# tomwhite/disq

Hardware: AMD Instinct MI355X
Metric: decompressed BAM GB/s + reads/sec (whole node) at 1/2/4/8 MI355X (higher is better)
Workload: dtype u8

## Files before the change

disq_amd/csrc/dq_hdr_core.h:

```cpp
#pragma once
#include <stdint.h>

#ifndef __HIPCC__
#ifndef __host__
#define __host__
#define __device__
#endif
#endif

#define DQH_INLINE __host__ __device__ inline __attribute__((always_inline))

namespace dqh {

enum : int32_t {
  HDR_NONE = 0,
  HDR_DYN = 1,
  HDR_ERR = 2,
};
constexpr int32_t HDR_BAD_TABLE = 4, HDR_OVERREAD = 8;
constexpr uint32_t HDR_WORDS = 160;
constexpr int HDR_LENS = 320;

struct HdrInfo {
  int32_t kind, status;
  int32_t nlen, ndist, bfinal;
  uint32_t end;
};

template <class Src>
struct Bits {
  uint64_t bb;
  uint32_t bc, wp;
  DQH_INLINE void init(const Src& S, uint32_t pos) {
    const uint32_t wi = pos >> 5, sh = pos & 31;
    bb = (((uint64_t)S.word(wi + 1) << 32) | S.word(wi)) >> sh;
    bc = 64 - sh;
    wp = wi + 2;
  }
  DQH_INLINE void fill(const Src& S) {
    if (bc <= 32) {
      bb |= (uint64_t)S.word(wp) << bc;
      bc += 32;
      wp += 1;
    }
  }
  DQH_INLINE uint32_t peek() const { return (uint32_t)bb; }
  DQH_INLINE void skip(uint32_t n) {
    bb >>= n;
    bc -= n;
  }
  DQH_INLINE uint32_t pos() const { return wp * 32 - bc; }
};

template <class Src, class Tbl, class Sink>
DQH_INLINE HdrInfo hdr_decode(const Src& S, Tbl& T, Sink& K, uint32_t pos, uint32_t endbits) {
  constexpr uint8_t order[19] = {16, 17, 18, 0, 8, 7, 9, 6, 10, 5, 11, 4, 12, 3, 13, 2, 14, 1, 15};
  HdrInfo R = {HDR_NONE, 0, 0, 0, 0, pos};
  if (pos + 3 > endbits) return R;
  Bits<Src> B;
  B.init(S, pos);
  const uint32_t h = B.peek();
  R.bfinal = (int32_t)(h & 1);
  if (((h >> 1) & 3) != 2) return R;
  R.nlen = (int32_t)((h >> 3) & 31) + 257;
  R.ndist = (int32_t)((h >> 8) & 31) + 1;
  const int ncode = (int)((h >> 13) & 15) + 4;
  B.skip(17);
  R.kind = HDR_ERR;
  R.status = HDR_BAD_TABLE;
  if (R.nlen > 286 || R.ndist > 30) return R;
  if (pos + 17 + 3 * (uint32_t)ncode > endbits) {
    R.status = HDR_OVERREAD;
    return R;
  }
  uint64_t cl = 0, cnt = 0;
  for (int i = 0; i < 19; i++) {
    B.fill(S);
    const uint32_t v = i < ncode ? B.peek() & 7 : 0;
    B.skip(i < ncode ? 3 : 0);
    cl |= (uint64_t)v << (3 * order[i]);
    cnt += 1ull << (8 * v);
  }
  uint64_t nxt = 0;
  {
    int left = 1;
    uint32_t code = 0;
    bool ok = true;
    for (int l = 1; l <= 7; l++) {
      const int c = (int)((cnt >> (8 * l)) & 0xff);
      left = 2 * left - c;
      ok = ok && left >= 0;
      nxt |= (uint64_t)(code & 0xff) << (8 * l);
      code = (code + (uint32_t)c) << 1;
    }
    if (!ok || left != 0) return R;
  }
  for (int s = 0; s < 19; s++) {
    const uint32_t l = (uint32_t)(cl >> (3 * s)) & 7;
    if (l == 0) continue;
    const uint32_t c = (uint32_t)(nxt >> (8 * l)) & 0xff;
    nxt += 1ull << (8 * l);
    uint32_t r = 0;
    for (uint32_t i = 0; i < l; i++) r |= ((c >> i) & 1u) << (l - 1 - i);
    for (uint32_t k = r & 127; k < 128; k += 1u << l) T.set(k, (uint32_t)s << 3 | l);
  }
  const int total = R.nlen + R.ndist;
  int have = 0, prev = -1;
  bool eob = false;
  for (int it = 0; it < 316 && have < total; it++) {
    if (B.pos() > endbits) {
      R.status = HDR_OVERREAD;
      return R;
    }
    B.fill(S);
    const uint32_t v = B.peek();
    const uint32_t e = T.get(v & 127);
    const uint32_t len = e & 7, sy = e >> 3;
    if (len == 0) return R;
    const uint32_t ex = sy < 16 ? 0u : sy == 16 ? 2u : sy == 17 ? 3u : 7u;
    const int xv = (int)((v >> len) & ((1u << ex) - 1));
    B.skip(len + ex);
    const int rep = sy < 16 ? 1 : sy == 18 ? 11 + xv : 3 + xv;
    const int val = sy < 16 ? (int)sy : sy == 16 ? prev : 0;
    if (val < 0) return R;
    if (have + rep > total) return R;
    if (val != 0)
      for (int i = have; i < have + rep; i++) {
        K.put((uint32_t)(i < R.nlen ? i : 288 + i - R.nlen), (uint32_t)val);
        eob = eob || i == 256;
      }
    have += rep;
    prev = val;
  }
  if (have < total) return R;
  R.end = B.pos();
  if (R.end > endbits) {
    R.status = HDR_OVERREAD;
    return R;
  }
  if (!eob) return R;
  R.kind = HDR_DYN;
  R.status = 0;
  return R;
}

}
```

disq_amd/csrc/dq_inflate3.hip:

```cpp
#include "dq_hdr_core.h"
#include "dq_inflate_core.h"
#include "dq_internal.h"

#include <mutex>
#include <vector>

namespace dq {
namespace {

using namespace dqi;

#define DQ_HD __device__ __host__ __attribute__((always_inline)) inline

#ifndef DQ_BLK_WG
#define DQ_BLK_WG 512
#endif
constexpr int WG = DQ_BLK_WG;
static_assert(WG % 128 == 0 && WG >= 512 && WG <= 1024, "whole waves on every SIMD");
constexpr int NWV = WG / 64;
constexpr int NDEC = WG;
constexpr uint32_t OV_DEFAULT = 96;
#ifndef DQ_TAIL_OV
#define DQ_TAIL_OV OV_DEFAULT
#endif
// ... 1370 lines not shown
    }
    int32_t msv[NE];
    uint32_t da[NB], db[NB];
#pragma unroll
    for (int k = 0; k < NB; k++) {
      const int32_t g0 = b0 + k * CH + G * t;
#pragma unroll
      for (int i = 0; i < G; i++) {
        const uint64_t mi = mw[k] & (~0ull >> (63 - ((g0 + i) & 63)));
        msv[k * G + i] = mi ? (g0 | 63) - (int32_t)__clzll(mi) : lsv[k];
      }
      da[k] = load_desc(L, sh + min(msv[k * G], 65535));
      db[k] = G > 1 ? load_desc(L, sh + min(msv[k * G + G - 1], 65535)) : da[k];
    }
#pragma unroll
    for (int k = 0; k < NB; k++) {
      const int32_t g0 = b0 + k * CH + G * t;
      const int32_t sbk = b0 + k * CH + (CSTEP ? 0 : ((G * t) & ~511));
#pragma unroll
      for (int i = 0; i < G; i++) {
        const int e = k * G + i;
        const int32_t x = g0 + i, ms = msv[e];
        const bool before = ms < b0;
        const uint32_t desc = before ? cdesc : (ms == msv[k * G + G - 1] ? db[k] : da[k]);
        const int32_t len = (int32_t)(desc >> 15) + 3, D1 = (int32_t)(desc & 0x7fff);
        const bool copy = x < rsize && ms != 0xffff && (!before || ms == cms) && x < ms + len;
        const int32_t jj = x - ms;
        int32_t src = (int32_t)((uint32_t)D1 ^ ~0u) + x;
        if (__builtin_expect(__any(copy && jj > D1), 0)) {
          const int32_t D = D1 + 1;
          const int32_t q = (int32_t)((float)jj * __builtin_amdgcn_rcpf((float)D));
          int32_t r = jj - q * D;
          r = r >= D ? r - D : r;
          src = ms - D + r;
        }
        DQ_CHK(!copy || (src >= 0 && src < x), CHK_K2_SRC);
        const bool done = !copy || src < sbk;
        fr[e] = copy ? src : x;
        xs[e] = done ? x : src;
        pending = pending || !done;
        nxt[x - b0] = (uint16_t)(copy ? src : x);
      }
    }
  };
  auto jump_round = [&](int32_t b0, int32_t* fr, int32_t* xs, bool& pending) {
    int32_t qv[NE];
#pragma unroll
    for (int e = 0; e < NE; e++) {
      DQ_CHK(xs[e] - b0 >= 0 && xs[e] - b0 < BATCH, CHK_K2_NXT);
      qv[e] = (int32_t)zx16(nxt[xs[e] - b0]);
    }
    bool any = false;
#pragma unroll
    for (int e = 0; e < NE; e++) {
      const int32_t own = (e / G) * CH + G * t + e % G;
      const int32_t p = xs[e], q = qv[e];
      const bool pd = p != b0 + own;
      const int32_t sbk = b0 + (e / G) * CH + (CSTEP ? 0 : ((G * t) & ~511));
      const bool fin = pd && (q == p || q < sbk);
      const bool go = pd && !fin;
      fr[e] = fin ? q : fr[e];
      xs[e] = go ? q : b0 + own;
      any = any || go;
      if constexpr (!QUAD) nxt[own] = (uint16_t)q;
    }
    if constexpr (QUAD) {
#pragma unroll
      for (int k = 0; k < NB; k++)
        store_nxt4(k * CH + 4 * t, pack16(qv[4 * k], qv[4 * k + 1]), pack16(qv[4 * k + 2], qv[4 * k + 3]));
    }
    pending = any;
  };
  constexpr bool SLICE = DQ_RES_SLICE != 0;
  const uint32_t own2 = 2u * (uint32_t)t;
  auto LB = [](int e) { return 2u << e; };
  auto nxt_at = [&](int e, uint32_t ra) {
    return reinterpret_cast<uint16_t*>(reinterpret_cast<char*>(nxt) + e * (CH * 2) + ra);
  };
  auto adopt_live = [&](int32_t b0, int32_t* fr, uint32_t* ra, uint32_t& live) {
    int32_t qv[NE];
#pragma unroll
    for (int e = 0; e < NE; e++) qv[e] = (int32_t)zx16(*nxt_at(e, own2));
    const uint32_t cb = 2u * (uint32_t)-b0;
    live = 0;
    uint64_t anym = 0;
#pragma unroll
    for (int e = 0; e < NE; e++) {
      const uint32_t na = ((uint32_t)qv[e] << 1) + (cb - 2u * e * CH);
      const bool pend = na < own2;
      fr[e] = qv[e];
      ra[e] = pend ? na : own2;
      if constexpr (SLICE) live |= __ballot(pend) != 0 ? LB(e) : 0u;
      else anym |= __ballot(pend);
    }
    if constexpr (!SLICE) live = anym != 0 ? LB(0) : 0u;
  };
  auto jump_round_live = [&](int32_t b0, int32_t* fr, uint32_t* ra, uint32_t& live) {
    const uint32_t cb = 2u * (uint32_t)-b0;
#pragma unroll
    for (int e = 0; e < NE; e++)
      if (!SLICE || (live & LB(e))) {
        DQ_CHK(ra[e] < 2u * CH && !(ra[e] & 1u), CHK_K2_NXT);
        fr[e] = *nxt_at(e, ra[e]);
      }
    uint32_t nl = 0;
    uint64_t anym = 0;
#pragma unroll
    for (int e = 0; e < NE; e++)
      if (!SLICE || (live & LB(e))) {
        const uint32_t q = zx32(fr[e]);
        fr[e] = (int32_t)q;
        const uint32_t na = (q << 1) + (cb - 2u * e * CH);
        const bool pd = ra[e] != own2, lt = na < ra[e];
        ra[e] = pd && lt ? na : own2;
        if constexpr (SLICE) nl |= (__ballot(pd) & __ballot(lt)) != 0 ? LB(e) : 0u;
        else anym |= __ballot(pd) & __ballot(lt);
        *nxt_at(e, own2) = (uint16_t)q;
      }
    live = SLICE ? nl : anym != 0 ? LB(0) : 0u;
  };
  int32_t frA[NE], xsA[NE];
  uint32_t raA[NE];
  bool pendA = false;
  uint32_t liveA = 0;
  auto left = [&](bool pending, uint32_t live) { return HYB ? live != 0 : pending; };
  auto round = [&](int32_t b0, int32_t* fr, int32_t* xs, uint32_t* ra, bool& pending, uint32_t& live) {
    if constexpr (HYB) jump_round_live(b0, fr, ra, live);
    else jump_round(b0, fr, xs, pending);
  };
  int32_t cms = -1;
  uint32_t cdesc = 0;
  first_hop(0, cms, cdesc, frA, xsA, pendA);
  if (t < (rsize + BATCH - 1) / BATCH) {
    int32_t ncms = -1;
    uint32_t ncdesc = 0;
    const int32_t x = (t + 1) * BATCH - 1;
    if (x + 1 < rsize) {
      const uint64_t m = bm64[x >> 6];
      const int32_t ms = m ? (x | 63) - (int32_t)__clzll(m) : (int32_t)L.u.r.last_start[(x >> 6) - 1];
      if (ms != 0xffff) {
        const uint32_t desc = load_desc(L, sh + ms);
        if (ms + (int32_t)(desc >> 15) + 3 > x + 1) {
          ncms = ms;
          ncdesc = desc;
        }
      }
    }
    L.u.r.carry_ms[t] = ncms;
    L.u.r.carry_desc[t] = ncdesc;
  }
  __syncthreads();
  if constexpr (HYB) adopt_live(0, frA, raA, liveA);
  for (int hop = 0; left(pendA, liveA) && hop < WG + 2; hop++) round(0, frA, xsA, raA, pendA, liveA);
  const int32_t rsize_u = HYB ? __builtin_amdgcn_readfirstlane(rsize) : rsize;
  for (int32_t bs = 0; bs < rsize_u; bs += BATCH) {
    const uint64_t tb0 = TIMING ? __builtin_amdgcn_s_memtime() : 0;
    const int32_t nbs = bs + BATCH;
    const bool more = nbs < rsize_u;
    __syncthreads();
    const int32_t ncms = more ? L.u.r.carry_ms[bs / BATCH] : -1;
    const uint32_t ncdesc = more ? L.u.r.carry_desc[bs / BATCH] : 0u;
    int32_t frB[NE], xsB[NE];
    uint32_t raB[NE];
    bool pendB = false;
    uint32_t liveB = 0;
    if (more) first_hop(nbs, ncms, ncdesc, frB, xsB, pendB);
    const uint64_t tb1 = TIMING ? __builtin_amdgcn_s_memtime() : 0;
#pragma unroll
    for (int k = 0; k < NB; k++) {
#pragma unroll
      for (int j = 0; j < (CSTEP ? 1 : G); j++) {
        const bool mine = CSTEP || ((G * t) >> 9) == j;
        const int32_t g0 = bs + k * CH + G * t;
        uint8_t v[G];
        if (mine)
#pragma unroll
          for (int i = 0; i < G; i++) {
            DQ_CHK(g0 + i >= rsize || (frA[k * G + i] >= 0 && frA[k * G + i] <= g0 + i), CHK_K2_SRC);
            v[i] = O[INR ? frA[k * G + i] : min(frA[k * G + i], 65535)];
          }
        if constexpr (HYB)
          if (k == 1 && more) adopt_live(nbs, frB, raB, liveB);
        if ((k > 0 || j > 0) && left(pendB, liveB)) round(nbs, frB, xsB, raB, pendB, liveB);
        if constexpr (QUAD && INR) {
          if (mine) {
            const uint32_t lo = (uint32_t)v[0] | (uint32_t)v[1] << 8;
            const uint32_t hi = (uint32_t)v[2] | (uint32_t)v[3] << 8;
            uint8_t* const p = L.out + sh + g0;
            if ((sh & 3) == 0) {
              const uint32_t w4 = lo | hi << 16;
              __builtin_memcpy(__builtin_assume_aligned(p, 4), &w4, 4);
            } else if ((sh & 3) == 2) {
              const uint16_t a2 = (uint16_t)lo, b2 = (uint16_t)hi;
              __builtin_memcpy(__builtin_assume_aligned(p, 2), &a2, 2);
              __builtin_memcpy(__builtin_assume_aligned(p + 2, 2), &b2, 2);
            } else {
              const uint16_t m2 = (uint16_t)(v[1] | v[2] << 8);
              p[0] = v[0];
              __builtin_memcpy(__builtin_assume_aligned(p + 1, 2), &m2, 2);
              p[3] = v[3];
            }
          }
        } else {
          if (mine)
#pragma unroll
            for (int i = 0; i < G; i++)
              if (g0 + i < rsize) L.out[sh + g0 + i] = v[i];
        }
        __syncthreads();
      }
    }
    if (left(pendB, liveB)) round(nbs, frB, xsB, raB, pendB, liveB);
    const uint64_t tb2 = TIMING ? __builtin_amdgcn_s_memtime() : 0;
    const int32_t c1 = min(rsize, nbs);
    const int32_t lines_to = c1 >= head ? (c1 - head) / 16 : 0;
    if (!(sflags & 1)) {
      for (int32_t k = lines_done + t; k < lines_to; k += WG) {
        const uint4 v = *reinterpret_cast<const uint4*>(O + head + 16 * k);
        uint4* d = reinterpret_cast<uint4*>(dstU + head + 16 * k);
        if (sflags & 2) st_nt(d, v);
        else *d = v;
      }
      lines_done = lines_to;
    }
    const uint64_t tb3 = TIMING ? __builtin_amdgcn_s_memtime() : 0;
    for (int hop = 0; left(pendB, liveB) && hop < WG + 2; hop++) round(nbs, frB, xsB, raB, pendB, liveB);
#pragma unroll
    for (int e = 0; e < NE; e++) frA[e] = frB[e];
    cms = ncms;
    cdesc = ncdesc;
    if (TIMING && t == 0) {
      tacc[9] += tb1 - tb0;
      tacc[12] += tb2 - tb1;
      tacc[13] += tb3 - tb2;
      tacc[14] += __builtin_amdgcn_s_memtime() - tb3;
      tacc[15] += 1;
    }
  }
  if (sflags & 1) {
    const int32_t lines_to = rsize >= head ? (rsize - head) / 16 : 0;
    for (int32_t k = t; k < lines_to; k += WG) {
      const uint4 v = *reinterpret_cast<const uint4*>(O + head + 16 * k);
      uint4* d = reinterpret_cast<uint4*>(dstU + head + 16 * k);
      if (sflags & 2) st_nt(d, v);
      else *d = v;
    }
    lines_done = lines_to;
  }
  uint32_t ct0 = 0, ct1 = 0, cshift = 0, cinit = 0, cwant = 0;
  if (verify_crc) {
    ct0 = (&c_crc4[0][0])[t];
    ct1 = t + WG < 1024 ? (&c_crc4[0][0])[t + WG] : 0u;
    cshift = c_slice_shift[WG - 1 - t];
    if (t == 0) {
      cinit = crc_init[rsize];
      const uint8_t* tr = C + cpos + csize - 8;
      cwant = (uint32_t)tr[0] | ((uint32_t)tr[1] << 8) | ((uint32_t)tr[2] << 16) | ((uint32_t)tr[3] << 24);
    }
  }
  static_assert(2 * WG >= 1024, "at most two CRC table words per thread");
  for (int x = t; x < head; x += WG) dstU[x] = O[x];
  for (int x = head + 16 * lines_done + t; x < rsize; x += WG) dstU[x] = O[x];
  TST(6);
  if (verify_crc) {
    __syncthreads();
    if (t < 1024) (&L.u.crc4[0][0])[t] = ct0;
    if (t + WG < 1024) (&L.u.crc4[0][0])[t + WG] = ct1;
    __syncthreads();
    const int32_t e = rsize - (WG - 1 - t) * CRC_SL;
    const int32_t s0 = max(0, e - CRC_SL);
    uint32_t cr = 0;
    if (e > 0) {
      int32_t x = s0;
      while (x < e && ((sh + x) & 3)) cr = L.u.crc4[0][(cr ^ O[x++]) & 0xff] ^ (cr >> 8);
      for (; x + 4 <= e; x += 4) {
        const uint32_t v = cr ^ *reinterpret_cast<const uint32_t*>(O + x);
        cr = L.u.crc4[3][v & 0xff] ^ L.u.crc4[2][(v >> 8) & 0xff] ^ L.u.crc4[1][(v >> 16) & 0xff] ^
             L.u.crc4[0][v >> 24];
      }
      while (x < e) cr = L.u.crc4[0][(cr ^ O[x++]) & 0xff] ^ (cr >> 8);
      cr = gf2_mulmod(cshift, cr);
    }
    cr = wave_incl_xor(cr);
    if (lane == 63) L.wsum[wv] = (int32_t)cr;
    __syncthreads();
    if (t == 0) {
      uint32_t x = 0;
      for (int w = 0; w < WG / 64; w++) x ^= (uint32_t)L.wsum[w];
      if (deferred) {
        tails[blockIdx.x].crc_raw = x;
      } else {
        const uint32_t crc = (x ^ cinit) ^ 0xffffffffu;
        if (crc != cwant) status[b] = ST_CRC;
      }
    }
  }
  TST(7);
  if (TIMING && t == 0)
    for (int i = 0; i < 24; i++) tim[(int64_t)blockIdx.x * TIM_W + i] = tacc[i];
  if (TIMING && t == 0)
    for (int i = 0; i < 7; i++) tim[(int64_t)blockIdx.x * TIM_W + 24 + i] = (uint64_t)L.misc[21 + i];
}

constexpr int HP_LS = 65;
struct HpSrc {
  const uint32_t* __restrict__ W;
  uint32_t last;
  DQ_AI uint32_t word(uint32_t i) const {
    return *reinterpret_cast<const uint32_t*>(reinterpret_cast<const uint8_t*>(W) + (min(i, last) << 2));
  }
};
struct HpTbl {
  uint8_t* t;
  DQ_AI void set(uint32_t k, uint32_t v) { t[k * 64] = (uint8_t)v; }
  DQ_AI uint32_t get(uint32_t k) const { return t[k * 64]; }
};
struct HpSink {
  uint32_t* w;
  uint32_t cur, acc;
  DQ_AI void put(uint32_t i, uint32_t v) {
    if ((i >> 3) != cur) {
      flush();
      cur = i >> 3;
      acc = 0;
    }
    acc |= v << (4 * (i & 7));
  }
  DQ_AI void flush() {
    if (acc) w[cur * HP_LS] = acc;
  }
};

template <bool TAIL>
__global__ __launch_bounds__(64) void inflate_header_kernel(
    const uint8_t* __restrict__ C, const int64_t* __restrict__ blk_pos,
    const int32_t* __restrict__ blk_csize, int64_t ngrid, const int32_t* __restrict__ sel,
    const TailDesc* __restrict__ tails, HdrMeta* __restrict__ hdr) {
  __shared__ uint8_t clt[128 * 64];
  __shared__ uint32_t lw[HDR_LW * HP_LS];
  const int lane = (int)threadIdx.x;
  const int64_t i0 = (int64_t)blockIdx.x * 64, i = i0 + lane;
  bool act = i < ngrid;
  uint32_t pos = 0;
  if (TAIL && act) {
    const TailDesc td = tails[i];
    act = td.flag == 1;
    pos = (uint32_t)td.pos;
  }
  for (int w = 0; w < HDR_LW; w++) lw[w * HP_LS + lane] = 0;
  dqh::HdrInfo R = {dqh::HDR_NONE, 0, 0, 0, 0, 0};
  if (act) {
    const int64_t b = sel ? (int64_t)sel[i] : i;
    const uint8_t* dp = C + blk_pos[b] + 18;
    const int mis = (int)(reinterpret_cast<uintptr_t>(dp) & 15);
    const uint32_t a0 = 8u * (uint32_t)mis;
    const uint32_t endbits = a0 + 8u * (uint32_t)max(blk_csize[b] - 26, 0);
    if (!TAIL) pos = a0;
    const HpSrc S{reinterpret_cast<const uint32_t*>(dp - mis), (pos >> 5) + dqh::HDR_WORDS - 1};
    HpTbl T{clt + lane};
    HpSink K{lw + lane, 0, 0};
    R = dqh::hdr_decode(S, T, K, pos, endbits);
    K.flush();
    HdrMeta m;
    m.info = (uint32_t)R.kind | (uint32_t)R.bfinal << 2 | (uint32_t)(R.ndist & 31) << 3 |
             (uint32_t)(R.nlen & 511) << 8 | (uint32_t)R.status << 24;
    m.end = R.end;
    m.pad[0] = m.pad[1] = 0;
    hdr[i] = m;
  }
  __syncthreads();
  const uint64_t dyn = __ballot(R.kind == dqh::HDR_DYN);
  uint32_t* out = reinterpret_cast<uint32_t*>(hdr + ngrid) + i0 * HDR_LW;
  for (int k = 0; k < HDR_LW; k++) {
    const int g = 64 * k + lane, r = g / HDR_LW, w = g - r * HDR_LW;
    if ((dyn >> r) & 1) out[g] = lw[w * HP_LS + r];
  }
}

struct alignas(16) LdsW {
  static constexpr int kLSUB = 0, kDROOT = 1 << LR, kDSUB = 0, kTEND = (1 << LR) + (1 << DR);
  static constexpr bool kPair = false;
  union {
    struct {
      uint16_t T[kTEND];
      HuffCanon hl, hd;
      uint16_t lend[16], dend[16];
      uint16_t lent[288];
      uint16_t dent[32];
      union {
        struct {
          uint8_t lens[320];
          uint8_t clen[20];
          uint16_t clt[128];
          int32_t cnt[32];
          int32_t run[32];
        } h;
      } x;
    } d;
    uint32_t crc4[4][256];
  } u;
  alignas(16) uint8_t out[TOUT + 32];
  alignas(8) uint32_t bm[TOUT / 32];
  uint32_t ck[T_NCK * 64];
  int32_t misc[8];
  uint32_t scratch[16];
};
static_assert(HB_WORDS * 4 <= LdsW::kTEND * 2, "header staging fits the decode table");
static_assert(4 * 4 * sizeof(LdsW) <= 160 * 1024, "four tails per workgroup, four workgroups per CU");
DQ_AI uint32_t* emit_dummy(LdsW& L) { return L.ck; }

DQ_AI uint32_t read_lengths_wave(LdsW& L, uint32_t P, int nlen, int ndist, uint32_t endbits,
                                 uint32_t hbase) {
  const uint32_t* hb = reinterpret_cast<const uint32_t*>(L.u.d.T);
  auto& H = L.u.d.x.h;
  const int lane = tid_fresh() & 63;
  const int total = nlen + ndist;
  int have = 0, prev = -1, entry = 0;
  for (uint32_t W0 = P;; W0 += 64) {
    if (W0 > endbits) {
      set_err(L, ST_OVERREAD);
      return W0;
    }
    const uint32_t p = W0 + (uint32_t)lane;
    const uint32_t wi = min((p >> 5) - hbase, (uint32_t)HB_WORDS - 2);
    const uint32_t v = (uint32_t)((((uint64_t)hb[wi + 1] << 32) | hb[wi]) >> (p & 31));
    const uint32_t ent = H.clt[v & 127];
    const uint32_t cl = ent & 7, sy = ent >> 3;
    const uint32_t ex = sy == 16 ? 2u : sy == 17 ? 3u : sy == 18 ? 7u : 0u;
    const int xv = (int)((v >> cl) & ((1u << ex) - 1));
    const int rep = sy < 16 ? 1 : sy == 16 ? 3 + xv : sy == 17 ? 3 + xv : 11 + xv;
    const int adv = cl ? (int)(cl + ex) : 0;
    int J[6];
    J[0] = adv ? min(lane + adv, 64) : lane;
#pragma unroll
    for (int k = 1; k < 6; k++) {
      const int y = __shfl(J[k - 1], J[k - 1] & 63, 64);
      J[k] = J[k - 1] >= 64 ? 64 : y;
    }
    int pk = entry;
#pragma unroll
    for (int k = 0; k < 6; k++) {
      const int y = __shfl(J[k], pk & 63, 64);
      if ((lane >> k) & 1) pk = pk >= 64 ? 64 : y;
    }
    const bool onp = pk < 64;
    const int src = pk & 63;
    const int s_rep = __shfl(rep, src, 64), s_adv = __shfl(adv, src, 64);
    const int s_sy = __shfl((int)sy, src, 64);
    const int pprev = __shfl_up(pk, 1, 64);
    const bool real = onp && (lane == 0 || pprev != pk);
    const bool bad = real && s_adv == 0;
    const int r = real && !bad ? s_rep : 0;
    const int incl = wave_incl_scan(r, lane);
    const int key = wave_incl_max(real && !bad && s_sy != 16 ? ((lane + 1) << 5) | (s_sy < 16 ? s_sy : 0) : 0);
    const int kprev = __shfl_up(key, 1, 64);
    const int before = lane == 0 ? 0 : kprev;
    const int val = s_sy < 16 ? s_sy : s_sy == 16 ? (before > 0 ? (before & 31) : prev) : 0;
    const bool take = real && have + incl - r < total;
    if (__any((take && bad) || (take && s_sy == 16 && val < 0) || (take && have + incl > total))) {
      set_err(L, ST_BAD_TABLE);
      return W0;
    }
    if (take && val != 0)
      for (int i = have + incl - r; i < have + incl; i++) H.lens[i < nlen ? i : 288 + i - nlen] = (uint8_t)val;
    const uint64_t tk = __ballot(take);
    const int lastk = tk ? 63 - (int)__clzll(tk) : -1;
    if (lastk >= 0 && __shfl(have + incl, lastk, 64) >= total) {
      __builtin_amdgcn_wave_barrier();
      return W0 + (uint32_t)__shfl(pk + s_adv, lastk, 64);
    }
    const uint64_t rm = __ballot(real);
    const int lastr = rm ? 63 - (int)__clzll(rm) : -1;
    if (lastr < 0 || __shfl((int)bad, lastr, 64)) {
      set_err(L, ST_BAD_TABLE);
      return W0;
    }
    have = __shfl(have + incl, lastr, 64);
    const int kl = __shfl(key, 63, 64);
    prev = kl > 0 ? (kl & 31) : prev;
    entry = __shfl(pk + s_adv, lastr, 64) - 64;
  }
}

DQ_AI void build_tables_wave(LdsW& L, int nlen, int ndist) {
  const int lane = tid_fresh() & 63;
  auto& H = L.u.d.x.h;
  if (lane < 32) {
    H.cnt[lane] = 0;
    H.run[lane] = 0;
  }
  __builtin_amdgcn_wave_barrier();
  for (int k = lane; k < 320; k += 64) {
    const bool isl = k < 288;
    const int len = isl ? (k < nlen ? H.lens[k] : 0) : (k - 288 < ndist ? H.lens[k] : 0);
    if (len) atomicAdd(&H.cnt[(isl ? 0 : 16) + len], 1);
  }
  __builtin_amdgcn_wave_barrier();
  __builtin_amdgcn_fence(__ATOMIC_SEQ_CST, "wavefront");
  int e = 0;
  {
    const int l = lane & 15;
    const bool in = lane < 32 && l >= 1;
    const int c = in ? H.cnt[lane] : 0;
    int offi = wave_incl_scan(c, lane);
    const int tt = in ? c << (16 - l) : 0;
    int cs = wave_incl_scan(tt, lane);
    const int base_o = __shfl(offi, 15, 64), base_c = __shfl(cs, 15, 64);
    if (lane >= 16) {
      offi -= base_o;
      cs -= base_c;
    }
    const int code = in ? (int)((uint32_t)(cs - tt) >> (16 - l)) : 0;
    const int left = in ? (1 << l) - (code + c) : 0;
    const bool isd = lane >= 16;
    HuffCanon& h = isd ? L.u.d.hd : L.u.d.hl;
    uint16_t* end = isd ? L.u.d.dend : L.u.d.lend;
    const int R = isd ? DR : LR;
    if (lane < 32) {
      h.first[l] = (uint16_t)code;
      h.count[l] = (uint16_t)c;
      h.offs[l] = (uint16_t)(offi - c);
      if (in && l <= R) end[l] = (uint16_t)((code + c) << (R - l));
    }
    const uint64_t over = __ballot(in && left < 0);
    const uint64_t used = __ballot(c > 0);
    const int left15l = __shfl(left, 15, 64), left15d = __shfl(left, 31, 64);
    const uint64_t ul = used & 0xffffull, ud = (used >> 16) & 0xffffull;
    const int maxll = ul ? 63 - __clzll(ul) : 0, maxld = ud ? 63 - __clzll(ud) : 0;
    if (over) e = ST_BAD_TABLE;
    if (maxll > 0 && left15l > 0 && maxll != 1) e = ST_BAD_TABLE;
    if (maxld > 0 && left15d > 0 && maxld != 1) e = ST_BAD_TABLE;
    const int ql0 = __shfl(offi, LR, 64), qln = __shfl(offi, 15, 64);
    const int qd0 = __shfl(offi, 16 + DR, 64), qdn = __shfl(offi, 31, 64);
    if (lane == 0) L.misc[M_SLOW] = (qln > ql0 || qdn > qd0) ? 1 : 0;
  }
  if (e) {
    if (lane == 0) set_err(L, e);
    return;
  }
  __builtin_amdgcn_wave_barrier();
  const uint64_t below = lanes_below(lane);
  for (int k0 = 0; k0 < 320; k0 += 64) {
    const int k = k0 + lane;
    const bool isl = k < 288;
    const int sym = isl ? k : k - 288;
    const int len = k < 320 ? (isl ? (k < nlen ? H.lens[k] : 0) : (sym < ndist ? H.lens[k] : 0)) : 0;
    const int key = (isl ? 0 : 16) + len;
    uint64_t peers = ~0ull;
#pragma unroll
    for (int bt = 0; bt < 5; bt++) {
      const uint64_t bl = __ballot((key >> bt) & 1);
      peers &= ((key >> bt) & 1) ? bl : ~bl;
    }
    const int run0 = H.run[key];
    const int rank = run0 + __popcll(peers & below);
    __builtin_amdgcn_wave_barrier();
    if (len && (peers >> lane) == 1ull) H.run[key] = run0 + __popcll(peers);
    if (len) {
      const HuffCanon& hh = isl ? L.u.d.hl : L.u.d.hd;
      const int q = hh.offs[len] + rank;
      if (isl) L.u.d.lent[q] = ent_ll((uint32_t)sym, (uint32_t)len);
      else L.u.d.dent[q] = ent_d((uint32_t)sym, (uint32_t)len);
    }
    __builtin_amdgcn_wave_barrier();
  }
  __builtin_amdgcn_wave_barrier();
  const bool lslow = L.u.d.hl.count[11] + L.u.d.hl.count[12] + L.u.d.hl.count[13] +
                         L.u.d.hl.count[14] + L.u.d.hl.count[15] > 0;
  const bool dslow = L.u.d.hd.count[9] + L.u.d.hd.count[10] + L.u.d.hd.count[11] + L.u.d.hd.count[12] +
                         L.u.d.hd.count[13] + L.u.d.hd.count[14] + L.u.d.hd.count[15] > 0;
#if DQ_ROOT_REG
  const RootEnds<LR> le = root_ends<LR>(L.u.d.lend);
  const RootEnds<DR> de = root_ends<DR>(L.u.d.dend);
#endif
  for (int i = lane; i < (1 << LR); i += 64) {
#if DQ_ROOT_REG
    const uint16_t v = root_entry_r<LR>(L.u.d.hl, le, L.u.d.lent, bitrev((uint32_t)i, LR));
#else
    const uint16_t v = root_entry<LR>(L, L.u.d.hl, L.u.d.lend, L.u.d.lent, bitrev((uint32_t)i, LR));
#endif
    L.u.d.T[i] = v ? v : lslow ? E_SLOW : (uint16_t)(LL_BAD | 1u);
  }
  for (int i = lane; i < (1 << DR); i += 64) {
#if DQ_ROOT_REG
    const uint16_t v = root_entry_r<DR>(L.u.d.hd, de, L.u.d.dent, bitrev((uint32_t)i, DR));
#else
    const uint16_t v = root_entry<DR>(L, L.u.d.hd, L.u.d.dend, L.u.d.dent, bitrev((uint32_t)i, DR));
#endif
    L.u.d.T[LdsW::kDROOT + i] = v ? v : dslow ? E_SLOW : (uint16_t)0x4001u;
  }
  __builtin_amdgcn_wave_barrier();
}

DQ_AI uint32_t x8n_tail(uint32_t n) {
  uint32_t p = 1u << 31;
  for (int k = 3; n; n >>= 1, k++)
    if (n & 1) p = gf2_mulmod(c_x2n[k & 31], p);
  return p;
}

template <bool TIMING>
__global__ __launch_bounds__(64 * TW, 4) void inflate_tail_kernel(
    const uint8_t* __restrict__ C, const int64_t* __restrict__ blk_pos,
    const int32_t* __restrict__ blk_csize, const int32_t* __restrict__ blk_usize,
    const int64_t* __restrict__ uoff, int64_t ngrid, uint8_t* __restrict__ U,
    int32_t* __restrict__ status, int32_t verify_crc, const uint32_t* __restrict__ crc_init,
    uint32_t OV, uint32_t sflags, const int32_t* __restrict__ sel,
    const TailDesc* __restrict__ tails, uint64_t* __restrict__ tim) {
  constexpr uint32_t CKI = CKI_DEFAULT;
  __shared__ LdsW Ls[TW];
  const int wv = __builtin_amdgcn_readfirstlane((int)(threadIdx.x >> 6)), lane = (int)(threadIdx.x & 63);
  const int64_t gi = (int64_t)blockIdx.x * TW + wv;
  if (gi >= ngrid) return;
  const TailDesc td = tails[gi];
  if (td.flag != 1) return;
  LdsW& L = Ls[wv];
  const uint64_t t0 = TIMING ? __builtin_amdgcn_s_memtime() : 0;
  const int64_t b = sel ? (int64_t)sel[gi] : gi;
  const int64_t cpos = blk_pos[b];
  const int32_t csize = blk_csize[b];
  const int32_t isize = blk_usize[b];
  const int64_t ub = uoff[b];
  const int32_t p0 = td.produced;
  const int sh = (int)((ub + p0) & 15);
  const uint8_t* dp = C + cpos + 18;
  const int mis = (int)(reinterpret_cast<uintptr_t>(dp) & 15);
  const uint32_t* W = reinterpret_cast<const uint32_t*>(__builtin_assume_aligned(dp - mis, 16));
  const int32_t dbytes = csize - 26;
  const uint32_t endbits = 8u * (uint32_t)mis + 8u * (uint32_t)max(dbytes, 0);
#ifdef DQ_CHECKED
  GSrc gsrc{W, (endbits >> 5) + 8, 4u << 12};
#else
  const GSrc gsrc{W};
#endif
  uint32_t warm = 0;
  {
    const uint32_t lo = (uint32_t)td.pos >> 3, nbytes = endbits / 8 - min(endbits / 8, lo);
    if ((uint32_t)lane * 128 < nbytes)
      warm = *reinterpret_cast<const uint32_t*>(reinterpret_cast<const uint8_t*>(W) + ((lo + 128 * lane) & ~3u));
  }
  for (int i = lane; i < TOUT / 32; i += 64) L.bm[i] = 0;
  if (lane < 8) L.misc[lane] = 0;
  uint32_t hinfo = 0, hend = 0;
  if (sflags & 32) {
    const HdrMeta* hdr = reinterpret_cast<const HdrMeta*>(tails + ngrid);
    const HdrMeta hm = hdr[gi];
    hinfo = hm.info;
    hend = hm.end;
    if (hm_kind(hinfo) == dqh::HDR_DYN && lane < HDR_LW) {
      const uint32_t w = reinterpret_cast<const uint32_t*>(hdr + ngrid)[gi * HDR_LW + lane];
      uint32_t* l8 = reinterpret_cast<uint32_t*>(L.u.d.x.h.lens);
      l8[2 * lane] = nib4(w & 0xffffu);
      l8[2 * lane + 1] = nib4(w >> 16);
    }
    if (hm_kind(hinfo) == dqh::HDR_ERR && lane == 0) L.misc[M_ERR] = hm_status(hinfo);
  }
  const bool hpre = hm_kind(hinfo) == dqh::HDR_DYN;
  __builtin_amdgcn_wave_barrier();
  int32_t produced = p0;
  uint32_t pos = (uint32_t)td.pos;
  uint64_t tph[5] = {0, 0, 0, 0, 0};
  uint64_t tl = TIMING ? __builtin_amdgcn_s_memtime() : 0;
  auto tick = [&](int k) {
    if (TIMING) {
      const uint64_t now = __builtin_amdgcn_s_memtime();
      tph[k] += now - tl;
      tl = now;
    }
  };
  while (L.misc[M_ERR] == 0 && produced < isize) {
    int nlen, ndist;
    int32_t bfinal;
    uint32_t a;
    if (hpre && pos == (uint32_t)td.pos) {
      nlen = hm_nlen(hinfo);
      ndist = hm_ndist(hinfo);
      bfinal = hm_bfinal(hinfo);
      a = hend;
// ... 495 lines not shown
```

Baseline: 197.8.

## Replace header LDS code-length table with register canonical lookup and staged input

The deflate dynamic-header kernel no longer builds a 128-entry code-length lookup table in LDS per lane. It decodes code-length symbols canonically from packed 64-bit register state, with a bit reverse and a compare over the length boundaries. The first 40 words of each block's bitstream are now loaded cooperatively into LDS with coalesced, shuffle-addressed loads, and only reads beyond that window go to global memory. The sink writes packed length nibbles in runs straight to global memory, replacing the LDS staging and ballot-based copy-out. This trades LDS traffic and table-fill work for more ALU work per symbol and uncoalesced direct global stores. The dropped len==0 check relies on the Kraft validation that runs earlier.

```diff
diff --git a/disq_amd/csrc/dq_hdr_core.h b/disq_amd/csrc/dq_hdr_core.h
--- a/disq_amd/csrc/dq_hdr_core.h
+++ b/disq_amd/csrc/dq_hdr_core.h
@@ -52,8 +52,30 @@
   DQH_INLINE uint32_t pos() const { return wp * 32 - bc; }
 };
 
-template <class Src, class Tbl, class Sink>
-DQH_INLINE HdrInfo hdr_decode(const Src& S, Tbl& T, Sink& K, uint32_t pos, uint32_t endbits) {
+DQH_INLINE uint32_t rev7(uint32_t v) {
+#ifdef __HIP_DEVICE_COMPILE__
+  return __builtin_bitreverse32(v) >> 25;
+#else
+  uint32_t r = 0;
+  for (int i = 0; i < 7; i++) r |= ((v >> i) & 1u) << (6 - i);
+  return r;
+#endif
+}
+
+struct ClCode {
+  uint64_t ends, off, lo, hi;
+  DQH_INLINE uint32_t lookup(uint32_t v) const {
+    const uint32_t rv = rev7(v);
+    uint32_t len = 1;
+    for (int l = 1; l <= 6; l++) len += ((uint32_t)(ends >> (8 * l)) & 0xffu) <= rv ? 1u : 0u;
+    const uint32_t q = ((rv >> (7 - len)) + (uint32_t)(off >> (8 * len))) & 31u;
+    const uint32_t sy = (uint32_t)(q < 12 ? lo >> (5 * q) : hi >> (5 * (q - 12))) & 31u;
+    return sy << 3 | len;
+  }
+};
+
+template <class Src, class Sink>
+DQH_INLINE HdrInfo hdr_decode(const Src& S, Sink& K, uint32_t pos, uint32_t endbits) {
   constexpr uint8_t order[19] = {16, 17, 18, 0, 8, 7, 9, 6, 10, 5, 11, 4, 12, 3, 13, 2, 14, 1, 15};
   HdrInfo R = {HDR_NONE, 0, 0, 0, 0, pos};
   if (pos + 3 > endbits) return R;
@@ -81,28 +103,31 @@
     cl |= (uint64_t)v << (3 * order[i]);
     cnt += 1ull << (8 * v);
   }
+  ClCode T = {0, 0, 0, 0};
   uint64_t nxt = 0;
   {
     int left = 1;
-    uint32_t code = 0;
+    uint32_t code = 0, q = 0;
     bool ok = true;
     for (int l = 1; l <= 7; l++) {
-      const int c = (int)((cnt >> (8 * l)) & 0xff);
-      left = 2 * left - c;
+      const uint32_t c = (uint32_t)(cnt >> (8 * l)) & 0xff;
+      left = 2 * left - (int)c;
       ok = ok && left >= 0;
-      nxt |= (uint64_t)(code & 0xff) << (8 * l);
-      code = (code + (uint32_t)c) << 1;
+      T.off |= (uint64_t)((q - code) & 0xff) << (8 * l);
+      nxt |= (uint64_t)q << (8 * l);
+      code += c;
+      q += c;
+      T.ends |= (uint64_t)((code << (7 - l)) & 0xff) << (8 * l);
+      code <<= 1;
     }
     if (!ok || left != 0) return R;
   }
   for (int s = 0; s < 19; s++) {
     const uint32_t l = (uint32_t)(cl >> (3 * s)) & 7;
-    if (l == 0) continue;
-    const uint32_t c = (uint32_t)(nxt >> (8 * l)) & 0xff;
+    const uint32_t p = (uint32_t)(nxt >> (8 * l)) & 0xff;
     nxt += 1ull << (8 * l);
-    uint32_t r = 0;
-    for (uint32_t i = 0; i < l; i++) r |= ((c >> i) & 1u) << (l - 1 - i);
-    for (uint32_t k = r & 127; k < 128; k += 1u << l) T.set(k, (uint32_t)s << 3 | l);
+    if (l != 0 && p < 12) T.lo |= (uint64_t)s << (5 * p);
+    if (l != 0 && p >= 12) T.hi |= (uint64_t)s << (5 * (p - 12));
   }
   const int total = R.nlen + R.ndist;
   int have = 0, prev = -1;
@@ -114,9 +139,8 @@
     }
     B.fill(S);
     const uint32_t v = B.peek();
-    const uint32_t e = T.get(v & 127);
+    const uint32_t e = T.lookup(v);
     const uint32_t len = e & 7, sy = e >> 3;
-    if (len == 0) return R;
     const uint32_t ex = sy < 16 ? 0u : sy == 16 ? 2u : sy == 17 ? 3u : 7u;
     const int xv = (int)((v >> len) & ((1u << ex) - 1));
     B.skip(len + ex);
@@ -124,11 +148,16 @@
     const int val = sy < 16 ? (int)sy : sy == 16 ? prev : 0;
     if (val < 0) return R;
     if (have + rep > total) return R;
-    if (val != 0)
-      for (int i = have; i < have + rep; i++) {
-        K.put((uint32_t)(i < R.nlen ? i : 288 + i - R.nlen), (uint32_t)val);
-        eob = eob || i == 256;
+    if (val != 0) {
+      eob = eob || (have <= 256 && 256 < have + rep);
+      for (int i = have, n = rep; n > 0;) {
+        const bool lit = i < R.nlen;
+        const int m = lit && R.nlen - i < n ? R.nlen - i : n;
+        K.run((uint32_t)(lit ? i : 288 + i - R.nlen), (uint32_t)m, (uint32_t)val);
+        i += m;
+        n -= m;
       }
+    }
     have += rep;
     prev = val;
   }
diff --git a/disq_amd/csrc/dq_inflate3.hip b/disq_amd/csrc/dq_inflate3.hip
--- a/disq_amd/csrc/dq_inflate3.hip
+++ b/disq_amd/csrc/dq_inflate3.hip
@@ -1696,32 +1696,38 @@
     for (int i = 0; i < 7; i++) tim[(int64_t)blockIdx.x * TIM_W + 24 + i] = (uint64_t)L.misc[21 + i];
 }
 
-constexpr int HP_LS = 65;
+constexpr int HP_LS = 65, HP_SW = 40;
+typedef const __attribute__((address_space(1))) uint32_t* hp_gptr;
+typedef const __attribute__((address_space(3))) uint32_t* hp_lptr;
 struct HpSrc {
-  const uint32_t* __restrict__ W;
-  uint32_t last;
+  hp_gptr W;
+  hp_lptr st;
+  uint32_t base;
   DQ_AI uint32_t word(uint32_t i) const {
-    return *reinterpret_cast<const uint32_t*>(reinterpret_cast<const uint8_t*>(W) + (min(i, last) << 2));
-  }
-};
-struct HpTbl {
-  uint8_t* t;
-  DQ_AI void set(uint32_t k, uint32_t v) { t[k * 64] = (uint8_t)v; }
-  DQ_AI uint32_t get(uint32_t k) const { return t[k * 64]; }
+    const uint32_t k = i - base;
+    uint32_t v = st[min(k, (uint32_t)HP_SW - 1) * HP_LS];
+    if (k >= (uint32_t)HP_SW) {
+      v = W[min(i, base + dqh::HDR_WORDS - 1)];
+      asm volatile("" : "+v"(v));
+    }
+    return v;
+  }
 };
 struct HpSink {
   uint32_t* w;
-  uint32_t cur, acc;
-  DQ_AI void put(uint32_t i, uint32_t v) {
-    if ((i >> 3) != cur) {
-      flush();
-      cur = i >> 3;
-      acc = 0;
-    }
-    acc |= v << (4 * (i & 7));
-  }
-  DQ_AI void flush() {
-    if (acc) w[cur * HP_LS] = acc;
+  uint32_t cur;
+  uint64_t acc;
+  DQ_AI void upto(uint32_t n) {
+#pragma clang loop vectorize(disable) unroll(disable)
+    while (cur < n) {
+      w[cur] = (uint32_t)acc;
+      acc >>= 32;
+      cur += 1;
+    }
+  }
+  DQ_AI void run(uint32_t i, uint32_t n, uint32_t v) {
+    upto(i >> 3);
+    acc |= (uint64_t)((0x111111u & ((1u << (4 * n)) - 1)) * v) << (4 * (i - 8 * cur));
   }
 };
 
@@ -1730,10 +1736,9 @@
     const uint8_t* __restrict__ C, const int64_t* __restrict__ blk_pos,
     const int32_t* __restrict__ blk_csize, int64_t ngrid, const int32_t* __restrict__ sel,
     const TailDesc* __restrict__ tails, HdrMeta* __restrict__ hdr) {
-  __shared__ uint8_t clt[128 * 64];
-  __shared__ uint32_t lw[HDR_LW * HP_LS];
+  __shared__ uint32_t st[HP_SW * HP_LS];
   const int lane = (int)threadIdx.x;
-  const int64_t i0 = (int64_t)blockIdx.x * 64, i = i0 + lane;
+  const int64_t i = (int64_t)blockIdx.x * 64 + lane;
   bool act = i < ngrid;
   uint32_t pos = 0;
   if (TAIL && act) {
@@ -1741,33 +1746,49 @@
     act = td.flag == 1;
     pos = (uint32_t)td.pos;
   }
-  for (int w = 0; w < HDR_LW; w++) lw[w * HP_LS + lane] = 0;
-  dqh::HdrInfo R = {dqh::HDR_NONE, 0, 0, 0, 0, 0};
+  const uint32_t* W = nullptr;
+  uint32_t endbits = 0;
   if (act) {
     const int64_t b = sel ? (int64_t)sel[i] : i;
     const uint8_t* dp = C + blk_pos[b] + 18;
     const int mis = (int)(reinterpret_cast<uintptr_t>(dp) & 15);
     const uint32_t a0 = 8u * (uint32_t)mis;
-    const uint32_t endbits = a0 + 8u * (uint32_t)max(blk_csize[b] - 26, 0);
+    endbits = a0 + 8u * (uint32_t)max(blk_csize[b] - 26, 0);
     if (!TAIL) pos = a0;
-    const HpSrc S{reinterpret_cast<const uint32_t*>(dp - mis), (pos >> 5) + dqh::HDR_WORDS - 1};
-    HpTbl T{clt + lane};
-    HpSink K{lw + lane, 0, 0};
-    R = dqh::hdr_decode(S, T, K, pos, endbits);
-    K.flush();
+    W = reinterpret_cast<const uint32_t*>(dp - mis);
+  }
+  {
+    const uintptr_t h = W ? reinterpret_cast<uintptr_t>(W + (pos >> 5)) : (reinterpret_cast<uintptr_t>(C) + 3) & ~(uintptr_t)3;
+    const int hlo = (int)(uint32_t)h, hhi = (int)(uint32_t)(h >> 32);
+    constexpr int B = 8;
+    static_assert(HP_SW % B == 0, "whole batches");
+    for (int k0 = 0; k0 < HP_SW; k0 += B) {
+      uint32_t v[B];
+#pragma unroll
+      for (int u = 0; u < B; u++) {
+        const int g = 64 * (k0 + u) + lane, r = g / HP_SW, j = g - r * HP_SW;
+        const uintptr_t q = (uintptr_t)(uint32_t)__shfl(hlo, r, 64) | (uintptr_t)(uint32_t)__shfl(hhi, r, 64) << 32;
+        v[u] = ((hp_gptr)q)[j];
+      }
+#pragma unroll
+      for (int u = 0; u < B; u++) {
+        const int g = 64 * (k0 + u) + lane, r = g / HP_SW, j = g - r * HP_SW;
+        st[j * HP_LS + r] = v[u];
+      }
+    }
+  }
+  __syncthreads();
+  if (act) {
+    const HpSrc S{(hp_gptr)W, (hp_lptr)(st + lane), pos >> 5};
+    HpSink K{reinterpret_cast<uint32_t*>(hdr + ngrid) + i * HDR_LW, 0, 0};
+    const dqh::HdrInfo R = dqh::hdr_decode(S, K, pos, endbits);
+    if (R.kind == dqh::HDR_DYN) K.upto(HDR_LW);
     HdrMeta m;
     m.info = (uint32_t)R.kind | (uint32_t)R.bfinal << 2 | (uint32_t)(R.ndist & 31) << 3 |
              (uint32_t)(R.nlen & 511) << 8 | (uint32_t)R.status << 24;
     m.end = R.end;
     m.pad[0] = m.pad[1] = 0;
     hdr[i] = m;
-  }
-  __syncthreads();
-  const uint64_t dyn = __ballot(R.kind == dqh::HDR_DYN);
-  uint32_t* out = reinterpret_cast<uint32_t*>(hdr + ngrid) + i0 * HDR_LW;
-  for (int k = 0; k < HDR_LW; k++) {
-    const int g = 64 * k + lane, r = g / HDR_LW, w = g - r * HDR_LW;
-    if ((dyn >> r) & 1) out[g] = lw[w * HP_LS + r];
   }
 }
 
```

New measurement: 199.0 (median of 6 runs). Within noise of the previous version (+0.6%).
